# zillow/salve

Hardware: AMD Instinct MI355X
Metric: alignment hypotheses/sec (render+verify) (higher is better)
Workload: dtype fp16

## Files before the change

### salve_amd/csrc/bev_render.hip

```cpp
#include <hip/hip_runtime.h>
#include <stdlib.h>
#include <stdint.h>
#include <stdio.h>
#include <string.h>

#include "../../include/salve_hip.h"
#if defined(SALVE_PROFILE_WALK)
enum { SDC_apex = 0, SDC_apex_slow, SDC_apex_far, SDC_rows, SDC_bits, SDC_exact, SDC_apex_table, SDC_apex_cached, SDC_N };
__shared__ int sd_counters[SDC_N];
#if defined(SALVE_PROFILE_NO_COUNT)
#define SD_COUNT(c)
#else
#define SD_COUNT(c) atomicAdd(&sd_counters[SDC_##c], 1)
#endif
enum { SDP_table = 0, SDP_window, SDP_share, SDP_slow, SDP_far, SDP_e2_total, SDP_e1_total, SDP_nearest, SDP_N };
__shared__ int sd_timers[SDP_N];
__shared__ int sd_phase[8];
#define SD_HARD_REASON(slot) atomicAdd(&sd_phase[slot], 1)
#define SD_PHASE(slot, t) { const long long now_ = clock64(); if ((threadIdx.x & 63) == 0) atomicAdd(&sd_phase[slot], (int)((now_ - (t)) >> 4)); (t) = now_; }
#define SD_NOW() clock64()
#define SD_LAP(slot, t) { const long long now_ = clock64(); if ((threadIdx.x & 63) == 0) atomicAdd(&sd_timers[SDP_##slot], (int)((now_ - (t)) >> 4)); (t) = now_; }
#endif
#include "star_delaunay.h"
#include "star_local.h"
#include "star_table.h"
#include <mutex>
#include "salve_common.h"

namespace {

constexpr int DENSIFY_THREADS = 512;
constexpr int MASK_ROWS_PER_TASK = 16;
constexpr int MASK_MAX_HALF = 8;
constexpr int N_SCAL = 24;
#ifndef SALVE_E2_GROUP
#define SALVE_E2_GROUP 64
#endif
#ifndef SALVE_HARD_RUN
#define SALVE_HARD_RUN 8
#endif
constexpr int E2_GROUP = SALVE_E2_GROUP;
constexpr int HARD_RUN = SALVE_HARD_RUN;
constexpr int KEY_SLICE_SHIFT = 21;
constexpr uint32_t KEY_INDEX_MASK = (1u << KEY_SLICE_SHIFT) - 1u;

struct DevCfg {
    int pano_h, pano_w, crop_rows, rows, npts;
    int H, W, wpr, mask_half;
    float depth_scale;
    double xmin, xmax, ymin, ymax, tx, ty, scale;
    double rp00, rp01, rp10, rp11;
    double zlo[2], zhi[2], zmin;
    int nslices;
    int out_flags;
    int dbg_flags;
};

struct DensifyCfg {
    int H, W, wpr, mask_half, out_flags, dbg_flags;
};

#include "bev_splat.h"

__global__ __launch_bounds__(256) void bev_scatter_points_kernel(DevCfg c, const double* __restrict__ xyz, int npts,
                                                                 uint32_t* __restrict__ kimg, int* __restrict__ n_in_window) {
    const int i = blockIdx.x * 256 + threadIdx.x;
    if (i >= npts) return;
    const double x1 = xyz[3 * (size_t)i], y1 = xyz[3 * (size_t)i + 1], z = xyz[3 * (size_t)i + 2];
    if (!(c.xmin <= x1 && x1 <= c.xmax && c.ymin <= y1 && y1 <= c.ymax)) return;
    atomicAdd(n_in_window, 1);
    const int ix = (int)rint((x1 + c.tx) * c.scale);
    const int iy = (int)rint((y1 + c.ty) * c.scale);
    const double zs = floor(z) - c.zmin;
    if (!(zs >= 0.0 && zs < (double)c.nslices) || ix < 0 || ix >= c.W || iy < 0 || iy >= c.H) return;
    atomicMax(kimg + (size_t)iy * c.W + ix, ((uint32_t)((int)zs + 1) << KEY_SLICE_SHIFT) | (uint32_t)i);
}

struct RasterEmit {
    int H, W, wpr;
    const uint32_t* occ;
    const uint32_t* msk;
    uint32_t* bev;
    int flip;
    int lane, nlanes;
    bool skip;
    int32_t* status;
    __device__ __forceinline__ uint32_t pix(int x, int y) const { return (uint32_t)(((flip >= 0 ? flip - y : y) * W) + x); }

    static __device__ __forceinline__ int floor_div(int n, int d, float inv_d) {
        int q = (int)floorf((float)n * inv_d);
        const int r = n - q * d;
        q += (r >= d) ? 1 : 0;
        q -= (r < 0) ? 1 : 0;
        return q;
    }

    static __device__ __forceinline__ uint32_t blend(int32_t wa, int32_t wb, int32_t wc, int32_t area, float inv_area, uint32_t ca,
                                                     uint32_t cb, uint32_t cc) {
        uint32_t out = 0;
#pragma unroll
        for (int ch = 0; ch < 3; ch++) {
            const uint32_t num = __umul24((uint32_t)wa, (ca >> (8 * ch)) & 255u) + __umul24((uint32_t)wb, (cb >> (8 * ch)) & 255u) +
                                 __umul24((uint32_t)wc, (cc >> (8 * ch)) & 255u);
            uint32_t q = (uint32_t)((float)num * inv_area);
            const int32_t r = (int32_t)(num - __umul24(q, (uint32_t)area));
            q += (r >= area) ? 1u : 0u;
            q -= (r < 0) ? 1u : 0u;
            out |= q << (8 * ch);
        }
        return out;
    }

    __device__ __forceinline__ void operator()(int ax, int ay, int bx, int by, int cx, int cy) const {
        const int32_t area = sd_orient(ax, ay, bx, by, cx, cy);
        if (area <= 1 || skip) return;
        int x0 = min(ax, min(bx, cx)), x1 = max(ax, max(bx, cx));
        const int y0 = min(ay, min(by, cy)), y1 = max(ay, max(by, cy));
        if ((x0 | y0) < 0 || x1 >= W || y1 >= H) {
            if (status && lane == 0) atomicOr(status, SALVE_STATUS_WALK_FAILED);
            return;
        }
        uint32_t ca = 0, cb = 0, cc = 0;
        bool have = false;
        const bool wide = (x1 - x0) > 40;
        const float inv_area = 1.0f / (float)area;
        const int ex[3][4] = {{bx, by, cx, cy}, {cx, cy, ax, ay}, {ax, ay, bx, by}};
        int eA[3], eB[3], eC[3];
        float einv[3];
#pragma unroll
        for (int e = 0; e < 3; e++) {
            const int px = ex[e][0], py = ex[e][1], qx = ex[e][2], qy = ex[e][3];
            eA[e] = -(qy - py);
            eB[e] = qx - px;
            eC[e] = (qy - py) * px - (qx - px) * py;
            einv[e] = eA[e] != 0 ? 1.0f / (float)(eA[e] < 0 ? -eA[e] : eA[e]) : 0.f;
        }
        for (int y = y0 + lane; y <= y1; y += nlanes) {
            int xa = x0, xb = x1;
            if (wide) {
                bool empty = false;
#pragma unroll
                for (int e = 0; e < 3; e++) {
                    const int32_t A = eA[e];
                    const int32_t D = eB[e] * y + eC[e];
                    if (A > 0) {
                        xa = max(xa, floor_div(-D + A - 1, A, einv[e]));
                    } else if (A < 0) {
                        xb = min(xb, floor_div(D, -A, einv[e]));
                    } else if (D < 0) {
                        empty = true;
                    }
                }
                if (empty || xa > xb) continue;
            }
            for (int w = xa >> 5; w <= (xb >> 5); w++) {
                uint32_t bits = msk[(y * wpr) + w] & ~occ[(y * wpr) + w];
                const int lo = xa - (w << 5), hi = xb - (w << 5);
                if (lo > 0) bits &= 0xFFFFFFFFu << lo;
                if (hi < 31) bits &= 0xFFFFFFFFu >> (31 - hi);
                while (bits) {
                    const int x = (w << 5) + (__ffs((int)bits) - 1);
                    bits &= bits - 1;
                    const int32_t wa = sd_orient(bx, by, cx, cy, x, y);
                    const int32_t wb = sd_orient(cx, cy, ax, ay, x, y);
                    const int32_t wc = area - wa - wb;
                    if ((wa | wb | wc) < 0) continue;
                    if (!have) {
                        ca = __hip_atomic_load(bev + pix(ax, ay), __ATOMIC_RELAXED, __HIP_MEMORY_SCOPE_AGENT);
                        cb = __hip_atomic_load(bev + pix(bx, by), __ATOMIC_RELAXED, __HIP_MEMORY_SCOPE_AGENT);
                        cc = __hip_atomic_load(bev + pix(cx, cy), __ATOMIC_RELAXED, __HIP_MEMORY_SCOPE_AGENT);
                        have = true;
                    }
                    bev[pix(x, y)] = blend(wa, wb, wc, area, inv_area, ca, cb, cc);
                }
            }
        }
    }
};

template <class T>
__device__ __forceinline__ void store_wb(T* p, T v) { *p = v; }

constexpr uint32_t HARD_FRESH = 1u << 22;
constexpr uint32_t HARD_SECOND = 1u << 23;
__device__ __forceinline__ void push_hard(uint32_t* list, int* counter, int cap, uint32_t site, uint32_t state, int32_t* status) {
    const int k = atomicAdd(counter, 1);
    if (k < cap) {
        *reinterpret_cast<uint2*>(list + 2 * k) = make_uint2(site, state);
    } else if (status) {
        atomicOr(status, SALVE_STATUS_WALK_FAILED);
    }
}

struct QueueEmit {
    unsigned long long* queue;
    int* counter;
    int capacity;
    bool drop;
    int32_t* status;
    __device__ __forceinline__ void operator()(int ax, int ay, int bx, int by, int cx, int cy) const {
        if (drop) return;
        const int32_t area = sd_orient(ax, ay, bx, by, cx, cy);
        if (area <= 1) return;
        const int slot = atomicAdd(counter, 1);
        if (slot < capacity) {
            const uint32_t rel = (uint32_t)((bx - ax) & 0xFF) | ((uint32_t)((by - ay) & 0xFF) << 8) |
                                 ((uint32_t)((cx - ax) & 0xFF) << 16) | ((uint32_t)((cy - ay) & 0xFF) << 24);
            store_wb(queue + slot, ((unsigned long long)rel << 32) | ((uint32_t)ay << 16) | (uint32_t)ax);
        } else if (status) {
            atomicOr(status, SALVE_STATUS_WALK_FAILED);
        }
    }
};

__device__ __forceinline__ void wg_barrier_after_global_stores() {
    asm volatile("s_waitcnt vmcnt(0)" ::: "memory");
    __syncthreads();
}

__device__ __forceinline__ uint16_t f32_to_f16(float f) { return __builtin_bit_cast(uint16_t, (_Float16)f); }
__device__ __forceinline__ void tile_pixel(const uint32_t* __restrict__ img, int W, const int4 cy, const int4 cx, const float* __restrict__ lut, float v[3]) {
    const uint32_t p00 = img[(size_t)cy.x * W + cx.x], p01 = img[(size_t)cy.x * W + cx.y];
    const uint32_t p10 = img[(size_t)cy.y * W + cx.x], p11 = img[(size_t)cy.y * W + cx.y];
#pragma unroll
    for (int ch = 0; ch < 3; ch++) {
        const int a = (p00 >> (8 * ch)) & 255, b = (p01 >> (8 * ch)) & 255;
        const int cc = (p10 >> (8 * ch)) & 255, d = (p11 >> (8 * ch)) & 255;
        const int S0 = a * cx.z + b * cx.w;
        const int S1 = cc * cx.z + d * cx.w;
        int r = (((cy.z * (S0 >> 4)) >> 16) + ((cy.w * (S1 >> 4)) >> 16) + 2) >> 2;
        r = min(max(r, 0), 255);
        v[ch] = lut[ch * 256 + r];
    }
}


struct TileFuse {
    const salve_tile_job_t* jobs_a;
    const salve_tile_job_t* jobs_b;
    const uint32_t* tiles_b;
    const int32_t* coef_y;
    const int32_t* coef_x;
    const float* lut;
    uint16_t* out;
    int32_t resize, crop, out_c, reserved;
};
__global__ void bev_tile_fuse_kernel(TileFuse t, TileFuse* dst) { *dst = t; }

__device__ SdTable d_star_table;

static int ensure_star_table() {
    static std::mutex mu;
    static unsigned long long uploaded = 0;
    static SdTable host_table;
    static int built = 0;
    std::lock_guard<std::mutex> lock(mu);
    int dev = 0;
    SALVE_HIP_CHECK(hipGetDevice(&dev));
    if (dev >= 0 && dev < 64 && ((uploaded >> dev) & 1ull)) return SALVE_OK;
    if (built == 0) built = sdt_build(&host_table) ? 1 : -1;
    if (built < 0) { salve_fail("star table construction could not be certified"); return SALVE_ERR_UNSUPPORTED; }
    SALVE_HIP_CHECK(hipMemcpyToSymbol(HIP_SYMBOL(d_star_table), &host_table, sizeof(SdTable)));
    if (dev >= 0 && dev < 64) uploaded |= 1ull << dev;
    return SALVE_OK;
}

__host__ __device__ inline size_t bitmap_words_hw(int H, int W) {
    return (size_t)2 * ((W + TILE_W - 1) / TILE_W) * ((H + TILE_H - 1) / TILE_H) * TILE_H * TILE_WORDS;
}
constexpr int DENSIFY_ORDERED = 256;
constexpr int DENSIFY_TILES = 512;
__host__ __device__ inline size_t tile_fuse_word(size_t n) { return (2 * n + 3) & ~(size_t)3; }
constexpr int ORDER_BINS = 1024;
constexpr int ORDER_MIN_RENDERS = 1025;

__global__ __launch_bounds__(1024) void bev_order_kernel(const int32_t* __restrict__ cost, int n, int32_t* __restrict__ order) {
// ... 131 lines not shown
#pragma unroll
        for (int off = 1; off < 64; off <<= 1) {
            const int v = __shfl_up(incl, off);
            if (lane >= off) incl += v;
        }
        if (lane == 63) list_wave_total[wave] = incl;
        __syncthreads();
        int base = incl - cnt;
        for (int w = 0; w < wave; w++) base += list_wave_total[w];
        if (tid == DENSIFY_THREADS - 1) scal[14] = base + cnt;
        for (int i = w_begin; i < w_end; i++) {
            uint32_t bits = sdl_walk_word(occ, H, wpr, i);
            const int y = i / wpr, xb = (i - y * wpr) << 5;
            while (bits) {
                const int x = xb + __ffs((int)bits) - 1;
                bits &= bits - 1u;
                store_wb(sitelist + base++, ((uint32_t)y << 16) | (uint32_t)x);
            }
        }
    }

    {
        const int ntask_rows = (H + MASK_ROWS_PER_TASK - 1) / MASK_ROWS_PER_TASK;
        const int ntasks = ntask_rows * wpr;
        uint32_t rows[MASK_ROWS_PER_TASK + 2 * MASK_MAX_HALF];
        const bool active = tid < ntasks;
        const int w = tid % wpr, yb = (tid / wpr) * MASK_ROWS_PER_TASK;
#pragma unroll
        for (int i = 0; i < MASK_ROWS_PER_TASK + 2 * MASK_MAX_HALF; i++) {
            const int y = yb - MASK_MAX_HALF + i;
            rows[i] = (active && y >= 0 && y < H && i >= MASK_MAX_HALF - p && i < MASK_ROWS_PER_TASK + MASK_MAX_HALF + p)
                          ? msk[y * wpr + w]
                          : 0u;
        }
        __syncthreads();
#pragma unroll
        for (int i = 0; i < MASK_ROWS_PER_TASK; i++) {
            const int y = yb + i;
            uint32_t v = 0;
#pragma unroll
            for (int d = -MASK_MAX_HALF; d <= MASK_MAX_HALF; d++)
                if (d >= -p && d <= p) v |= rows[i + MASK_MAX_HALF + d];
            if (active && y < H) msk[y * wpr + w] = v;
        }
    }
    __syncthreads();

    if (c.out_flags & 2) {
        for (int i = tid; i < H * wpr; i += DENSIFY_THREADS) msk[i] = 0xFFFFFFFFu;
        __syncthreads();
    }
    const int nsites = scal[14];
    const bool degenerate = scal[0] < 4 || scal[1] == scal[2] || scal[3] <= 1;

    wg_barrier_after_global_stores();
    __builtin_amdgcn_fence(__ATOMIC_ACQUIRE, "agent");

#if defined(SALVE_PROFILE_WALK)
    SD_PHASE(0, t_phase);
#endif
    if (!degenerate && !(dbg_flags & 1)) {
        SdGrid g = {H, W, wpr, occ, rmin, rmax, 0, 1, (dbg_flags & 32) ? nullptr : &d_star_table.off[0][0][0], scal[1], scal[2], scal[12], scal[13], (H <= 1024 && W <= 1024 && !(dbg_flags & 256)) ? tri_cache : nullptr};
        RasterEmit raster = {H, W, wpr, occ, msk, bev, flip, 0, 1, (dbg_flags & 2) != 0, status};
        QueueEmit qemit = {triq, &scal[8], H * W, (dbg_flags & 1024) != 0, status};
        const int hard_cap = (H * W) >> 1;
        SdLean st;
        bool active = false, exhausted = false;
        int iters = 0;
        for (;;) {
            const unsigned long long idle = __ballot(!active && !exhausted);
            const unsigned long long busy = __ballot(active);
            if (idle != 0ull && (__popcll(idle) >= 16 || busy == 0ull)) {
                if (!active && !exhausted) {
                    const int i = atomicAdd(&scal[6], 1);
                    if (i >= nsites) {
                        exhausted = true;
                    } else {
                        const uint32_t s = __hip_atomic_load(sitelist + i, __ATOMIC_RELAXED, __HIP_MEMORY_SCOPE_AGENT);
                        if (dbg_stats) { atomicAdd(&scal[9], 1); atomicAdd(&scal[10], (int)(s & 0xFFFFu) + (int)(s >> 16)); }
                        if (sdl_lean_begin(st, g, (int)(s & 0xFFFFu), (int)(s >> 16)) == SDL_LEAN_CONTINUE) active = true;
                        else push_hard(hardlist, &scal[7], hard_cap, s, HARD_FRESH, status);
                    }
                }
            } else if (busy == 0ull) {
                break;
            }
            if (active) {
                const int r = sdl_lean_step(st, g, qemit);
                iters++;
                if (r != SDL_LEAN_CONTINUE) {
                    active = false;
                    if (dbg_mask && (dbg_flags & 16))
                    {
                        dbg_mask[((size_t)rid * H + st.sy) * W + st.sx] = (uint8_t)((r == SDL_LEAN_HARD ? 200 : 100) + min(st.deg, 50));
                    }
                    if (r == SDL_LEAN_HARD)
                        push_hard(hardlist, &scal[7], hard_cap, ((uint32_t)st.sy << 16) | (uint32_t)st.sx,
                                  (uint32_t)((st.ax + 128) & 0xFF) | ((uint32_t)((st.ay + 128) & 0xFF) << 8) | ((uint32_t)(st.n0x + 1) << 16) |
                                      ((uint32_t)(st.n0y + 1) << 18) | (st.dir > 0 ? 1u << 20 : 0u) | (st.half ? 1u << 21 : 0u) | (st.dir & 1 ? 0u : HARD_SECOND), status);
                }
            }
        }
        if (dbg_stats) atomicAdd(&scal[4], iters);
#if defined(SALVE_PROFILE_WALK)
        SD_PHASE(5, t_phase);
#endif
        wg_barrier_after_global_stores();
#if defined(SALVE_PROFILE_WALK)
        SD_PHASE(1, t_phase);
#endif
        const int nhard = min(scal[7], hard_cap);
        const int nq = min(scal[8], H * W);
        int err = 0;
#if defined(SALVE_PROFILE_WALK)
        long long t_e2 = SD_NOW();
#endif
        {
            SdGrid gw = g;
            gw.lane = lane & (E2_GROUP - 1);
            gw.nlanes = E2_GROUP;
            gw.gbase = lane & ~(E2_GROUP - 1);
            RasterEmit rw = raster;
            rw.lane = gw.lane;
            rw.nlanes = E2_GROUP;
            const int nh = (dbg_flags & 4) ? 0 : nhard;
            for (;;) {
                int i0 = 0;
                if (gw.lane == 0) i0 = atomicAdd(&scal[11], HARD_RUN);
                i0 = __shfl(i0, gw.gbase);
                if (i0 >= nh) break;
                static_assert(2 * HARD_RUN <= E2_GROUP, "a run's entries are fetched by one load of the group");
                uint32_t run_words = 0;
                if (gw.lane < 2 * HARD_RUN && 2 * i0 + gw.lane < 2 * nh)
                    run_words = __hip_atomic_load(hardlist + 2 * i0 + gw.lane, __ATOMIC_RELAXED, __HIP_MEMORY_SCOPE_AGENT);
                for (int i = i0; i < min(i0 + HARD_RUN, nh); i++) {
                    const uint32_t s = (uint32_t)__shfl((int)run_words, gw.gbase + 2 * (i - i0));
                    const uint32_t w = (uint32_t)__shfl((int)run_words, gw.gbase + 2 * (i - i0) + 1);
                    const int hx = (int)(s & 0xFFFFu), hy = (int)(s >> 16);
                    const int r = sd_walk(gw, hx, hy, (w & HARD_FRESH) != 0, (int)(w & 0xFF) - 128, (int)((w >> 8) & 0xFF) - 128, ((w >> 20) & 1u ? 1 : -1) * ((w & HARD_SECOND) ? 2 : 1),
                                          ((w >> 21) & 1u) != 0, (int)((w >> 16) & 3u) - 1, (int)((w >> 18) & 3u) - 1, rw);
                    if (r < 0) err = 1;
                }
            }
        }
#if defined(SALVE_PROFILE_WALK)
        SD_LAP(e2_total, t_e2);
        SD_PHASE(2, t_phase);
#endif
        if (err) {
            atomicOr(&scal[5], 1);
            if (status && (lane & (E2_GROUP - 1)) == 0) atomicOr(status, SALVE_STATUS_WALK_FAILED);
        }
        uint32_t* genlist = sitelist;
        for (int i = tid; i < ((dbg_flags & 8) ? 0 : nq); i += DENSIFY_THREADS) {
            const unsigned long long e = __hip_atomic_load(triq + i, __ATOMIC_RELAXED, __HIP_MEMORY_SCOPE_AGENT);
            const int ax = (int)(e & 0xFFFFu), ay = (int)((e >> 16) & 0xFFFFu);
            const uint32_t rel = (uint32_t)(e >> 32);
            const int bx = ax + (int8_t)(rel & 0xFF), by = ay + (int8_t)((rel >> 8) & 0xFF), cx = ax + (int8_t)((rel >> 16) & 0xFF), cy = ay + (int8_t)(rel >> 24);
            const int32_t area = sd_orient(ax, ay, bx, by, cx, cy);
            const bool centroid = area == 3 && (ax + bx + cx) % 3 == 0 && (ay + by + cy) % 3 == 0;
            if (area != 2 && !centroid) {
                store_wb(genlist + atomicAdd(&scal[15], 1), (uint32_t)i);
                continue;
            }
            if (dbg_flags & 2) continue;
            if (area == 2) {
                int px = cx, py = cy, qx = ax, qy = ay;
                if ((((bx - ax) | (by - ay)) & 1) == 0) { px = ax; py = ay; qx = bx; qy = by; }
                else if ((((cx - bx) | (cy - by)) & 1) == 0) { px = bx; py = by; qx = cx; qy = cy; }
                const int mx = (px + qx) >> 1, my = (py + qy) >> 1;
                if (!(((msk[(my * wpr) + (mx >> 5)] & ~occ[(my * wpr) + (mx >> 5)]) >> (mx & 31)) & 1u)) continue;
                const uint32_t cp = __hip_atomic_load(bev + pixi(px, py), __ATOMIC_RELAXED, __HIP_MEMORY_SCOPE_AGENT);
                const uint32_t cq = __hip_atomic_load(bev + pixi(qx, qy), __ATOMIC_RELAXED, __HIP_MEMORY_SCOPE_AGENT);
                bev[pixi(mx, my)] = (((cp & 0xFEFEFEu) >> 1) + ((cq & 0xFEFEFEu) >> 1) + (cp & cq & 0x010101u));
            } else {
                const int mx = (ax + bx + cx) / 3, my = (ay + by + cy) / 3;
                if (!(((msk[(my * wpr) + (mx >> 5)] & ~occ[(my * wpr) + (mx >> 5)]) >> (mx & 31)) & 1u)) continue;
                const uint32_t ca = __hip_atomic_load(bev + pixi(ax, ay), __ATOMIC_RELAXED, __HIP_MEMORY_SCOPE_AGENT);
                const uint32_t cb = __hip_atomic_load(bev + pixi(bx, by), __ATOMIC_RELAXED, __HIP_MEMORY_SCOPE_AGENT);
                const uint32_t cc = __hip_atomic_load(bev + pixi(cx, cy), __ATOMIC_RELAXED, __HIP_MEMORY_SCOPE_AGENT);
                uint32_t out = 0;
#pragma unroll
                for (int ch = 0; ch < 3; ch++) {
                    const uint32_t sum = ((ca >> (8 * ch)) & 255u) + ((cb >> (8 * ch)) & 255u) + ((cc >> (8 * ch)) & 255u);
                    out |= ((sum * 0xAAABu) >> 17) << (8 * ch);
                }
                bev[pixi(mx, my)] = out;
            }
        }
        wg_barrier_after_global_stores();
        const int ngen = min(scal[15], H * W);
        for (int i = tid; i < ngen; i += DENSIFY_THREADS) {
            const uint32_t qi = __hip_atomic_load(genlist + i, __ATOMIC_RELAXED, __HIP_MEMORY_SCOPE_AGENT);
            const unsigned long long e = __hip_atomic_load(triq + qi, __ATOMIC_RELAXED, __HIP_MEMORY_SCOPE_AGENT);
            const int ax = (int)(e & 0xFFFFu), ay = (int)((e >> 16) & 0xFFFFu);
            const uint32_t rel = (uint32_t)(e >> 32);
            raster(ax, ay, ax + (int8_t)(rel & 0xFF), ay + (int8_t)((rel >> 8) & 0xFF), ax + (int8_t)((rel >> 16) & 0xFF),
                   ay + (int8_t)(rel >> 24));
        }
    }
    wg_barrier_after_global_stores();
#if defined(SALVE_PROFILE_WALK)
    SD_PHASE(3, t_phase);
#endif
    for (int i = tid; i < H * wpr; i += DENSIFY_THREADS) {
        uint32_t bits = occ[i] & (degenerate ? 0xFFFFFFFFu : ~msk[i]);
        const int y = i / wpr, xb = (i % wpr) << 5;
        while (bits) {
            const int x = xb + __ffs((int)bits) - 1;
            bits &= bits - 1u;
            bev[pixi(x, y)] = 0u;
        }
    }
    if (c.out_flags & DENSIFY_TILES) {
        wg_barrier_after_global_stores();
        asm volatile("buffer_inv sc1" ::: "memory");
        const TileFuse* tfp = reinterpret_cast<const TileFuse*>(reinterpret_cast<const int32_t*>(bitmaps_all + (size_t)gridDim.x * bitmap_words_hw(H, W)) + tile_fuse_word(gridDim.x));
        const TileFuse tf = *tfp;
        const salve_tile_job_t ja = tf.jobs_a[rid], jb = tf.jobs_b[rid];
        if (ja.slot >= 0) {
            int4* cy_l = reinterpret_cast<int4*>(smem);
            int4* cx_l = cy_l + tf.resize;
            float* lut_l = reinterpret_cast<float*>(cx_l + tf.resize);
            for (int i = tid; i < tf.resize; i += DENSIFY_THREADS) {
                cy_l[i] = reinterpret_cast<const int4*>(tf.coef_y)[i];
                cx_l[i] = reinterpret_cast<const int4*>(tf.coef_x)[i];
            }
            for (int i = tid; i < 3 * 256; i += DENSIFY_THREADS) lut_l[i] = tf.lut[i];
            __syncthreads();
            const int crop = tf.crop, off = (tf.resize - crop) / 2, out_c = tf.out_c;
            const bool a_first = ja.chan < jb.chan;
            const int c0 = a_first ? ja.chan : jb.chan;
            const uint32_t* tb = tf.tiles_b + jb.bev_offset;
            uint16_t* osample = tf.out + (size_t)ja.slot * crop * crop * out_c;
            constexpr int COLS = 256, RGROUPS = DENSIFY_THREADS / COLS;
            for (int j0 = 0; j0 < crop; j0 += COLS) {
                const int j = j0 + (tid & (COLS - 1));
                if (j >= crop) continue;
                const int4 cx = cx_l[j + off];
#ifndef SALVE_TILE_ROWS_IN_FLIGHT
#define SALVE_TILE_ROWS_IN_FLIGHT 8
#endif
                constexpr int U = SALVE_TILE_ROWS_IN_FLIGHT;
                for (int i0 = tid / COLS; i0 < crop; i0 += RGROUPS * U) {
                    int4 cy[U];
                    uint32_t p00[U], p01[U], p10[U], p11[U], q[U];
#pragma unroll
                    for (int u = 0; u < U; u++) {
                        const int i = min(i0 + u * RGROUPS, crop - 1);
                        cy[u] = cy_l[i + off];
                        const uint32_t* r0 = bev + __umul24(cy[u].x, W);
                        const uint32_t* r1 = bev + __umul24(cy[u].y, W);
                        p00[u] = r0[cx.x]; p01[u] = r0[cx.y]; p10[u] = r1[cx.x]; p11[u] = r1[cx.y];
                        q[u] = tb[i * crop + j];
                    }
#pragma unroll
                    for (int u = 0; u < U; u++) {
                        const int i = i0 + u * RGROUPS;
                        if (i >= crop) break;
                        const int idx = i * crop + j;
                        float va[3], vb[3];
#pragma unroll
                        for (int ch = 0; ch < 3; ch++) {
                            const uint32_t a = (p00[u] >> (8 * ch)) & 255u, b = (p01[u] >> (8 * ch)) & 255u;
                            const uint32_t cc = (p10[u] >> (8 * ch)) & 255u, d = (p11[u] >> (8 * ch)) & 255u;
                            const int S0 = (int)(__umul24(a, cx.z) + __umul24(b, cx.w));
                            const int S1 = (int)(__umul24(cc, cx.z) + __umul24(d, cx.w));
                            int r = (int)(((__umul24(cy[u].z, S0 >> 4) >> 16) + (__umul24(cy[u].w, S1 >> 4) >> 16) + 2u) >> 2);
                            r = min(max(r, 0), 255);
                            va[ch] = lut_l[ch * 256 + r];
                            vb[ch] = lut_l[ch * 256 + ((q[u] >> (8 * ch)) & 255u)];
                        }
                        const float* lo = a_first ? va : vb;
                        const float* hi = a_first ? vb : va;
                        typedef float f2 __attribute__((ext_vector_type(2)));
                        typedef _Float16 h2 __attribute__((ext_vector_type(2)));
                        const uint32_t w0 = __builtin_bit_cast(uint32_t, __builtin_convertvector((f2){lo[0], lo[1]}, h2));
                        const uint32_t w1 = __builtin_bit_cast(uint32_t, __builtin_convertvector((f2){lo[2], hi[0]}, h2));
                        const uint32_t w2 = __builtin_bit_cast(uint32_t, __builtin_convertvector((f2){hi[1], hi[2]}, h2));
                        uint16_t* px = osample + (size_t)idx * out_c;
                        if (out_c == 8) {
                            *reinterpret_cast<uint4*>(px) = make_uint4(w0, w1, w2, 0u);
                        } else {
                            uint32_t* o = reinterpret_cast<uint32_t*>(px + c0);
                            o[0] = w0; o[1] = w1; o[2] = w2;
                            if (c0 + 12 > out_c)
                                for (int k = c0 + 6; k < out_c; k += 2) *reinterpret_cast<uint32_t*>(px + k) = 0u;
                        }
                    }
                }
            }
        }
    }
    if (dbg_mask) {
        for (int i = tid; i < H * W; i += DENSIFY_THREADS) {
            const int y = i / W, x = i % W;
            dbg_mask[(size_t)rid * H * W + i] = (uint8_t)((msk[y * wpr + (x >> 5)] >> (x & 31)) & 1u);
        }
    }
    if (dbg_stats) {
        __syncthreads();
#if defined(SALVE_PROFILE_WALK)
        SD_PHASE(4, t_phase);
        __syncthreads();
        if (tid < 8) dbg_stats[rid * 8 + tid] = (dbg_flags & 128) ? sd_phase[tid] : (dbg_flags & 64) ? sd_timers[tid] : sd_counters[tid];
#else
        if (tid < 8) dbg_stats[rid * 8 + tid] = tid == 1 ? scal[9] : (tid == 2 ? scal[10] : (tid < 6 ? scal[tid] : scal[tid + 1]));
#endif
    }
}


__global__ __launch_bounds__(256) void bev_tile_kernel(const uint32_t* __restrict__ bev, int W,
                                                       const salve_tile_job_t* __restrict__ jobs,
                                                       const int32_t* __restrict__ coef_y,
                                                       const int32_t* __restrict__ coef_x, int resize, int crop,
                                                       const float* __restrict__ lut, void* __restrict__ out, int fmt,
                                                       int out_c) {
    const salve_tile_job_t job = jobs[blockIdx.y];
    const int idx = blockIdx.x * 256 + threadIdx.x;
    if (idx >= crop * crop) return;
    const int i = idx / crop, j = idx % crop;
    const int off = (resize - crop) / 2;
    const int4 cy = reinterpret_cast<const int4*>(coef_y)[i + off];
    const int4 cx = reinterpret_cast<const int4*>(coef_x)[j + off];
    const uint32_t* img = bev + job.bev_offset;
    const uint32_t p00 = img[(size_t)cy.x * W + cx.x], p01 = img[(size_t)cy.x * W + cx.y];
    const uint32_t p10 = img[(size_t)cy.y * W + cx.x], p11 = img[(size_t)cy.y * W + cx.y];
    float v[3];
    int rq[3];
#pragma unroll
    for (int ch = 0; ch < 3; ch++) {
        const int a = (p00 >> (8 * ch)) & 255, b = (p01 >> (8 * ch)) & 255;
        const int cc = (p10 >> (8 * ch)) & 255, d = (p11 >> (8 * ch)) & 255;
        const int S0 = a * cx.z + b * cx.w;
        const int S1 = cc * cx.z + d * cx.w;
        int r = (((cy.z * (S0 >> 4)) >> 16) + ((cy.w * (S1 >> 4)) >> 16) + 2) >> 2;
        r = min(max(r, 0), 255);
        rq[ch] = r;
        v[ch] = lut[ch * 256 + r];
    }
    if (fmt == SALVE_TILE_U8X4) {
        reinterpret_cast<uint32_t*>(out)[(size_t)job.slot * crop * crop + idx] = (uint32_t)rq[0] | ((uint32_t)rq[1] << 8) | ((uint32_t)rq[2] << 16);
    } else if (fmt == SALVE_TILE_F32_NCHW) {
        float* o = reinterpret_cast<float*>(out) + ((size_t)job.slot * out_c + job.chan) * crop * crop + idx;
#pragma unroll
        for (int ch = 0; ch < 3; ch++) o[(size_t)ch * crop * crop] = v[ch];
    } else {
        uint16_t* o = reinterpret_cast<uint16_t*>(out) + ((size_t)job.slot * crop * crop + idx) * out_c + job.chan;
#pragma unroll
        for (int ch = 0; ch < 3; ch++) o[ch] = f32_to_f16(v[ch]);
// ... 714 lines not shown
```

### salve_amd/csrc/star_local.h

```cpp
#pragma once
#include "star_delaunay.h"
#include "star_table.h"

#define SDL_XLO (-16)
#define SDL_NONE 0x7FFF

SD_FN uint32_t sdl_row32(const SdGrid& g, int y, int x0) {
    const bool yin = (unsigned)y < (unsigned)g.H;
    const int w0 = x0 >> 5, sh = x0 & 31;
    const bool in0 = yin & ((unsigned)w0 < (unsigned)g.wpr), in1 = yin & ((unsigned)(w0 + 1) < (unsigned)g.wpr);
    const int base = SD_MUL(yin ? y : 0, g.wpr);
    uint32_t lo = g.occ[base + (in0 ? w0 : 0)], hi = g.occ[base + (in1 ? w0 + 1 : 0)];
    lo = in0 ? lo : 0u;
    hi = in1 ? hi : 0u;
#if defined(__HIP_DEVICE_COMPILE__)
    return __builtin_amdgcn_alignbit(hi, lo, (uint32_t)sh);
#else
    return sh ? ((lo >> sh) | (hi << (32 - sh))) : lo;
#endif
}

SD_FN bool sdl_bit(const SdGrid& g, int x, int y) {
    const bool in = (unsigned)x < (unsigned)g.W && (unsigned)y < (unsigned)g.H;
    const int xi = in ? x : 0, yi = in ? y : 0;
    return in & (bool)((g.occ[SD_MUL(yi, g.wpr) + (xi >> 5)] >> (xi & 31)) & 1u);
}

SD_FN uint32_t sdl_surrounded_word(uint32_t c, uint32_t l, uint32_t r, uint32_t uc) {
    const uint32_t right = (c >> 1) | (r << 31), left = (c << 1) | (l >> 31);
    return c & right & left & uc;
}
SD_FN uint32_t sdl_walk_word(const uint32_t* occ, int H, int wpr, int i) {
    const int y = i / wpr, w = i - y * wpr;
    const uint32_t c = occ[i];
    if (c == 0u || y + 1 >= H) return c;
    const uint32_t l = w > 0 ? occ[i - 1] : 0u, r = w + 1 < wpr ? occ[i + 1] : 0u;
    return c & ~sdl_surrounded_word(c, l, r, occ[i + wpr]);
}

enum { SDL_LEAN_CONTINUE = 0, SDL_LEAN_DONE = 1, SDL_LEAN_HARD = 2 };
#ifndef SD_HARD_REASON
#define SD_HARD_REASON(slot)
#endif

struct SdLean {
    int sx, sy;
    int n0x, n0y, ax, ay;
    int dir, deg;
    int round;
    bool half;
    bool aup;
};

SD_FN int sdl_lean_begin(SdLean& s, const SdGrid& g, int sx, int sy) {
    s.sx = sx;
    s.sy = sy;
    s.deg = 0;
    s.dir = 1;
    s.round = 0;
    s.half = false;
    s.aup = false;
    s.n0x = s.n0y = s.ax = s.ay = 0;
    if (g.tab == nullptr) return SDL_LEAN_HARD;
    const uint32_t c = sdl_row32(g, sy, sx + SDL_XLO), u = sdl_row32(g, sy + 1, sx + SDL_XLO), d = sdl_row32(g, sy - 1, sx + SDL_XLO);
    const int o = 0 - SDL_XLO;
    int nx = SDL_NONE, ny = 0;
    if ((d >> (o + 1)) & 1u) { nx = 1; ny = -1; }
    if ((d >> (o - 1)) & 1u) { nx = -1; ny = -1; }
    if ((u >> (o - 1)) & 1u) { nx = -1; ny = 1; }
    if ((u >> (o + 1)) & 1u) { nx = 1; ny = 1; }
    if ((d >> o) & 1u) { nx = 0; ny = -1; }
    if ((u >> o) & 1u) { nx = 0; ny = 1; }
    if ((c >> (o - 1)) & 1u) { nx = -1; ny = 0; }
    if ((c >> (o + 1)) & 1u) { nx = 1; ny = 0; }
    s.half = ((c >> (o + 1)) & 1u) != 0;
    s.n0x = s.ax = nx;
    s.n0y = s.ay = ny;
    const bool n0up = ny > 0 || s.half;
    s.aup = n0up;
    s.dir = s.half ? 2 : ((!n0up && nx < 0) ? -1 : 1);
    return nx == SDL_NONE ? SDL_LEAN_HARD : SDL_LEAN_CONTINUE;
}

template <class Emit>
SD_FN int sdl_lean_step(SdLean& s, const SdGrid& g, Emit& emit) {
    const int ox = s.dir > 0 ? 0 : s.ax, oy = s.dir > 0 ? 0 : s.ay;
    const int vx = s.dir > 0 ? s.ax : -s.ax, vy = s.dir > 0 ? s.ay : -s.ay;
    int px = SDL_NONE, py = 0;
    if (vx >= -SDT_AMAX && vx <= SDT_AMAX && vy >= -SDT_AMAX && vy <= SDT_AMAX) {
        const uint32_t* row = (const uint32_t*)(g.tab + sdt_index(vx, vy) * (SDT_LEN * 2));
        const int bx = s.sx + ox, by = s.sy + oy;
        const int k = s.round;
        const uint32_t e0 = row[2 * k], e1 = row[2 * k + 1];
        const int x0 = (int8_t)(e0 & 0xFF), y0 = (int8_t)((e0 >> 8) & 0xFF), x1 = (int8_t)((e0 >> 16) & 0xFF), y1 = (int8_t)(e0 >> 24);
        const int x2 = (int8_t)(e1 & 0xFF), y2 = (int8_t)((e1 >> 8) & 0xFF), x3 = (int8_t)((e1 >> 16) & 0xFF), y3 = (int8_t)(e1 >> 24);
        const bool b0 = sdl_bit(g, bx + x0, by + y0), b1 = sdl_bit(g, bx + x1, by + y1);
        const bool b2 = sdl_bit(g, bx + x2, by + y2), b3 = sdl_bit(g, bx + x3, by + y3);
        if (b0 | b1 | b2 | b3) {
            px = ox + (b0 ? x0 : b1 ? x1 : b2 ? x2 : x3);
            py = oy + (b0 ? y0 : b1 ? y1 : b2 ? y2 : y3);
        } else if (k + 1 < SDT_LEAN_LEN / 4) {
            s.round = k + 1;
            return SDL_LEAN_CONTINUE;
        }
    }
    s.round = 0;
    const bool second = (s.dir & 1) == 0, aup = s.aup;
    const bool n0up = s.n0y > 0;
    const bool fin = second | (aup & !n0up);
    bool sw;
    bool up = aup;
    if (px == SDL_NONE) {
        if (!sd_side_is_empty(g, s.sx, s.sy, s.sx + s.ax, s.sy + s.ay, s.dir)) {
            SD_HARD_REASON((vx >= -SDT_AMAX && vx <= SDT_AMAX && vy >= -SDT_AMAX && vy <= SDT_AMAX) ? 7 : 6);
            return SDL_LEAN_HARD;
        }
        if (fin) return SDL_LEAN_DONE;
        sw = true;
    } else {
        const bool pup = sd_before(0, 0, px, py);
        if (aup & pup) {
            if (s.dir > 0) emit(s.sx, s.sy, s.sx + s.ax, s.sy + s.ay, s.sx + px, s.sy + py);
            else emit(s.sx, s.sy, s.sx + px, s.sy + py, s.sx + s.ax, s.sy + s.ay);
        }
        sw = aup & !pup;
        if (sw ? fin : (!second && px == s.n0x && py == s.n0y)) return SDL_LEAN_DONE;
        up = pup;
    }
    if (sw) {
        s.dir = s.dir > 0 ? -2 : 2;
        px = s.n0x;
        py = s.n0y;
        up = n0up;
    }
    s.aup = up;
    s.ax = px;
    s.ay = py;
    if (++s.deg > 64) return SDL_LEAN_HARD;
    return SDL_LEAN_CONTINUE;
}
```

Baseline: 60370.

## Batch densify and raster triangle loads to keep several in flight

Restructures the densify loop and the general-triangle raster loop so each thread handles several triangles per iteration. It issues all queue and pixel-color loads up front before doing any compute or stores, which hides global memory latency. The raster functor gains a templated path that accepts prefetched vertex colors. Separately, the lean star-walk step is rewritten with early returns to simplify control flow. The cost is higher register pressure and extra clamped or dummy loads at the loop tails.

```diff
diff --git a/salve_amd/csrc/bev_render.hip b/salve_amd/csrc/bev_render.hip
--- a/salve_amd/csrc/bev_render.hip
+++ b/salve_amd/csrc/bev_render.hip
@@ -41,6 +41,10 @@
 #endif
 constexpr int E2_GROUP = SALVE_E2_GROUP;
 constexpr int HARD_RUN = SALVE_HARD_RUN;
+#ifndef SALVE_RASTER_TRIS_IN_FLIGHT
+#define SALVE_RASTER_TRIS_IN_FLIGHT 4
+#endif
+constexpr int RASTER_TRIS = SALVE_RASTER_TRIS_IN_FLIGHT;
 constexpr int KEY_SLICE_SHIFT = 21;
 constexpr uint32_t KEY_INDEX_MASK = (1u << KEY_SLICE_SHIFT) - 1u;
 
@@ -111,7 +115,14 @@
         return out;
     }
 
-    __device__ __forceinline__ void operator()(int ax, int ay, int bx, int by, int cx, int cy) const {
+    __device__ __forceinline__ void operator()(int ax, int ay, int bx, int by, int cx, int cy) const { run<false>(ax, ay, bx, by, cx, cy, 0u, 0u, 0u); }
+
+    __device__ __forceinline__ bool inside(int ax, int ay, int bx, int by, int cx, int cy) const {
+        return (min(ax, min(bx, cx)) | min(ay, min(by, cy))) >= 0 && max(ax, max(bx, cx)) < W && max(ay, max(by, cy)) < H;
+    }
+
+    template <bool FETCHED>
+    __device__ __forceinline__ void run(int ax, int ay, int bx, int by, int cx, int cy, uint32_t ca, uint32_t cb, uint32_t cc) const {
         const int32_t area = sd_orient(ax, ay, bx, by, cx, cy);
         if (area <= 1 || skip) return;
         int x0 = min(ax, min(bx, cx)), x1 = max(ax, max(bx, cx));
@@ -120,8 +131,7 @@
             if (status && lane == 0) atomicOr(status, SALVE_STATUS_WALK_FAILED);
             return;
         }
-        uint32_t ca = 0, cb = 0, cc = 0;
-        bool have = false;
+        bool have = FETCHED;
         const bool wide = (x1 - x0) > 40;
         const float inv_area = 1.0f / (float)area;
         const int ex[3][4] = {{bx, by, cx, cy}, {cx, cy, ax, ay}, {ax, ay, bx, by}};
@@ -559,51 +569,113 @@
             if (status && (lane & (E2_GROUP - 1)) == 0) atomicOr(status, SALVE_STATUS_WALK_FAILED);
         }
         uint32_t* genlist = sitelist;
-        for (int i = tid; i < ((dbg_flags & 8) ? 0 : nq); i += DENSIFY_THREADS) {
-            const unsigned long long e = __hip_atomic_load(triq + i, __ATOMIC_RELAXED, __HIP_MEMORY_SCOPE_AGENT);
-            const int ax = (int)(e & 0xFFFFu), ay = (int)((e >> 16) & 0xFFFFu);
-            const uint32_t rel = (uint32_t)(e >> 32);
-            const int bx = ax + (int8_t)(rel & 0xFF), by = ay + (int8_t)((rel >> 8) & 0xFF), cx = ax + (int8_t)((rel >> 16) & 0xFF), cy = ay + (int8_t)(rel >> 24);
-            const int32_t area = sd_orient(ax, ay, bx, by, cx, cy);
-            const bool centroid = area == 3 && (ax + bx + cx) % 3 == 0 && (ay + by + cy) % 3 == 0;
-            if (area != 2 && !centroid) {
-                store_wb(genlist + atomicAdd(&scal[15], 1), (uint32_t)i);
-                continue;
-            }
-            if (dbg_flags & 2) continue;
-            if (area == 2) {
-                int px = cx, py = cy, qx = ax, qy = ay;
-                if ((((bx - ax) | (by - ay)) & 1) == 0) { px = ax; py = ay; qx = bx; qy = by; }
-                else if ((((cx - bx) | (cy - by)) & 1) == 0) { px = bx; py = by; qx = cx; qy = cy; }
-                const int mx = (px + qx) >> 1, my = (py + qy) >> 1;
+        constexpr int U = RASTER_TRIS;
+        enum { TRI_NONE = 0, TRI_MIDPOINT = 1, TRI_CENTROID = 2, TRI_GENERAL = 3 };
+        const int nqf = (dbg_flags & 8) ? 0 : nq;
+        for (int i0 = tid; i0 < nqf; i0 += U * DENSIFY_THREADS) {
+            unsigned long long e[U];
+#pragma unroll
+            for (int u = 0; u < U; u++) {
+                const int i = i0 + u * DENSIFY_THREADS;
+                e[u] = __hip_atomic_load(triq + min(i, nqf - 1), __ATOMIC_RELAXED, __HIP_MEMORY_SCOPE_AGENT);
+            }
+            int kind[U];
+            uint32_t ca[U], cb[U], cc[U], dst[U];
+#pragma unroll
+            for (int u = 0; u < U; u++) {
+                const int ax = (int)(e[u] & 0xFFFFu), ay = (int)((e[u] >> 16) & 0xFFFFu);
+                const uint32_t rel = (uint32_t)(e[u] >> 32);
+                const int bx = ax + (int8_t)(rel & 0xFF), by = ay + (int8_t)((rel >> 8) & 0xFF), cx = ax + (int8_t)((rel >> 16) & 0xFF), cy = ay + (int8_t)(rel >> 24);
+                const int32_t area = sd_orient(ax, ay, bx, by, cx, cy);
+                const bool centroid = area == 3 && (ax + bx + cx) % 3 == 0 && (ay + by + cy) % 3 == 0;
+                kind[u] = TRI_NONE;
+                ca[u] = cb[u] = cc[u] = dst[u] = 0u;
+                if (i0 + u * DENSIFY_THREADS >= nqf) continue;
+                if (area != 2 && !centroid) {
+                    kind[u] = TRI_GENERAL;
+                    continue;
+                }
+                if (dbg_flags & 2) continue;
+                int mx, my;
+                if (area == 2) {
+                    int px = cx, py = cy, qx = ax, qy = ay;
+                    if ((((bx - ax) | (by - ay)) & 1) == 0) { px = ax; py = ay; qx = bx; qy = by; }
+                    else if ((((cx - bx) | (cy - by)) & 1) == 0) { px = bx; py = by; qx = cx; qy = cy; }
+                    mx = (px + qx) >> 1; my = (py + qy) >> 1;
+                    ca[u] = pixi(px, py); cb[u] = pixi(qx, qy);
+                } else {
+                    mx = (ax + bx + cx) / 3; my = (ay + by + cy) / 3;
+                    ca[u] = pixi(ax, ay); cb[u] = pixi(bx, by); cc[u] = pixi(cx, cy);
+                }
                 if (!(((msk[(my * wpr) + (mx >> 5)] & ~occ[(my * wpr) + (mx >> 5)]) >> (mx & 31)) & 1u)) continue;
-                const uint32_t cp = __hip_atomic_load(bev + pixi(px, py), __ATOMIC_RELAXED, __HIP_MEMORY_SCOPE_AGENT);
-                const uint32_t cq = __hip_atomic_load(bev + pixi(qx, qy), __ATOMIC_RELAXED, __HIP_MEMORY_SCOPE_AGENT);
-                bev[pixi(mx, my)] = (((cp & 0xFEFEFEu) >> 1) + ((cq & 0xFEFEFEu) >> 1) + (cp & cq & 0x010101u));
-            } else {
-                const int mx = (ax + bx + cx) / 3, my = (ay + by + cy) / 3;
-                if (!(((msk[(my * wpr) + (mx >> 5)] & ~occ[(my * wpr) + (mx >> 5)]) >> (mx & 31)) & 1u)) continue;
-                const uint32_t ca = __hip_atomic_load(bev + pixi(ax, ay), __ATOMIC_RELAXED, __HIP_MEMORY_SCOPE_AGENT);
-                const uint32_t cb = __hip_atomic_load(bev + pixi(bx, by), __ATOMIC_RELAXED, __HIP_MEMORY_SCOPE_AGENT);
-                const uint32_t cc = __hip_atomic_load(bev + pixi(cx, cy), __ATOMIC_RELAXED, __HIP_MEMORY_SCOPE_AGENT);
-                uint32_t out = 0;
+                kind[u] = area == 2 ? TRI_MIDPOINT : TRI_CENTROID;
+                dst[u] = pixi(mx, my);
+            }
+#pragma unroll
+            for (int u = 0; u < U; u++) {
+                if (kind[u] == TRI_MIDPOINT || kind[u] == TRI_CENTROID) {
+                    ca[u] = __hip_atomic_load(bev + ca[u], __ATOMIC_RELAXED, __HIP_MEMORY_SCOPE_AGENT);
+                    cb[u] = __hip_atomic_load(bev + cb[u], __ATOMIC_RELAXED, __HIP_MEMORY_SCOPE_AGENT);
+                }
+                if (kind[u] == TRI_CENTROID) cc[u] = __hip_atomic_load(bev + cc[u], __ATOMIC_RELAXED, __HIP_MEMORY_SCOPE_AGENT);
+            }
+            uint32_t out[U];
+#pragma unroll
+            for (int u = 0; u < U; u++) {
+                const uint32_t mid = (((ca[u] & 0xFEFEFEu) >> 1) + ((cb[u] & 0xFEFEFEu) >> 1) + (ca[u] & cb[u] & 0x010101u));
+                uint32_t third = 0;
 #pragma unroll
                 for (int ch = 0; ch < 3; ch++) {
-                    const uint32_t sum = ((ca >> (8 * ch)) & 255u) + ((cb >> (8 * ch)) & 255u) + ((cc >> (8 * ch)) & 255u);
-                    out |= ((sum * 0xAAABu) >> 17) << (8 * ch);
+                    const uint32_t sum = ((ca[u] >> (8 * ch)) & 255u) + ((cb[u] >> (8 * ch)) & 255u) + ((cc[u] >> (8 * ch)) & 255u);
+                    third |= ((sum * 0xAAABu) >> 17) << (8 * ch);
                 }
-                bev[pixi(mx, my)] = out;
+                out[u] = kind[u] == TRI_CENTROID ? third : mid;
+                asm volatile("" : "+v"(out[u]));
+            }
+#pragma unroll
+            for (int u = 0; u < U; u++) {
+                if (kind[u] == TRI_GENERAL) store_wb(genlist + atomicAdd(&scal[15], 1), (uint32_t)(i0 + u * DENSIFY_THREADS));
+                else if (kind[u] != TRI_NONE) bev[dst[u]] = out[u];
             }
         }
         wg_barrier_after_global_stores();
         const int ngen = min(scal[15], H * W);
-        for (int i = tid; i < ngen; i += DENSIFY_THREADS) {
-            const uint32_t qi = __hip_atomic_load(genlist + i, __ATOMIC_RELAXED, __HIP_MEMORY_SCOPE_AGENT);
-            const unsigned long long e = __hip_atomic_load(triq + qi, __ATOMIC_RELAXED, __HIP_MEMORY_SCOPE_AGENT);
-            const int ax = (int)(e & 0xFFFFu), ay = (int)((e >> 16) & 0xFFFFu);
-            const uint32_t rel = (uint32_t)(e >> 32);
-            raster(ax, ay, ax + (int8_t)(rel & 0xFF), ay + (int8_t)((rel >> 8) & 0xFF), ax + (int8_t)((rel >> 16) & 0xFF),
-                   ay + (int8_t)(rel >> 24));
+        for (int i0 = tid; i0 < ngen; i0 += U * DENSIFY_THREADS) {
+            uint32_t qi[U];
+            unsigned long long e[U];
+            uint32_t ca[U], cb[U], cc[U];
+#pragma unroll
+            for (int u = 0; u < U; u++)
+                qi[u] = __hip_atomic_load(genlist + min(i0 + u * DENSIFY_THREADS, ngen - 1), __ATOMIC_RELAXED, __HIP_MEMORY_SCOPE_AGENT);
+#pragma unroll
+            for (int u = 0; u < U; u++) e[u] = __hip_atomic_load(triq + qi[u], __ATOMIC_RELAXED, __HIP_MEMORY_SCOPE_AGENT);
+#pragma unroll
+            for (int u = 0; u < U; u++)
+                if (i0 + u * DENSIFY_THREADS >= ngen) e[u] = 0ull;
+#pragma unroll
+            for (int u = 0; u < U; u++) {
+                const int ax = (int)(e[u] & 0xFFFFu), ay = (int)((e[u] >> 16) & 0xFFFFu);
+                const uint32_t rel = (uint32_t)(e[u] >> 32);
+                const int bx = ax + (int8_t)(rel & 0xFF), by = ay + (int8_t)((rel >> 8) & 0xFF), cx = ax + (int8_t)((rel >> 16) & 0xFF), cy = ay + (int8_t)(rel >> 24);
+                ca[u] = cb[u] = cc[u] = 0u;
+                if (i0 + u * DENSIFY_THREADS < ngen && raster.inside(ax, ay, bx, by, cx, cy)) {
+                    ca[u] = __hip_atomic_load(bev + raster.pix(ax, ay), __ATOMIC_RELAXED, __HIP_MEMORY_SCOPE_AGENT);
+                    cb[u] = __hip_atomic_load(bev + raster.pix(bx, by), __ATOMIC_RELAXED, __HIP_MEMORY_SCOPE_AGENT);
+                    cc[u] = __hip_atomic_load(bev + raster.pix(cx, cy), __ATOMIC_RELAXED, __HIP_MEMORY_SCOPE_AGENT);
+                }
+            }
+#pragma unroll 1
+            for (int u = 0; u < U; u++) {
+                unsigned long long eu = e[0];
+                uint32_t cau = ca[0], cbu = cb[0], ccu = cc[0];
+#pragma unroll
+                for (int k = 1; k < U; k++)
+                    if (u == k) { eu = e[k]; cau = ca[k]; cbu = cb[k]; ccu = cc[k]; }
+                const int ax = (int)(eu & 0xFFFFu), ay = (int)((eu >> 16) & 0xFFFFu);
+                const uint32_t rel = (uint32_t)(eu >> 32);
+                raster.run<true>(ax, ay, ax + (int8_t)(rel & 0xFF), ay + (int8_t)((rel >> 8) & 0xFF), ax + (int8_t)((rel >> 16) & 0xFF),
+                                 ay + (int8_t)(rel >> 24), cau, cbu, ccu);
+            }
         }
     }
     wg_barrier_after_global_stores();
diff --git a/salve_amd/csrc/star_local.h b/salve_amd/csrc/star_local.h
--- a/salve_amd/csrc/star_local.h
+++ b/salve_amd/csrc/star_local.h
@@ -4,6 +4,9 @@
 
 #define SDL_XLO (-16)
 #define SDL_NONE 0x7FFF
+#ifndef SALVE_LEAN_EARLY_RETURN
+#define SALVE_LEAN_EARLY_RETURN 1
+#endif
 
 SD_FN uint32_t sdl_row32(const SdGrid& g, int y, int x0) {
     const bool yin = (unsigned)y < (unsigned)g.H;
@@ -108,6 +111,36 @@
     const bool second = (s.dir & 1) == 0, aup = s.aup;
     const bool n0up = s.n0y > 0;
     const bool fin = second | (aup & !n0up);
+#if SALVE_LEAN_EARLY_RETURN
+    if (px == SDL_NONE) {
+        if (!sd_side_is_empty(g, s.sx, s.sy, s.sx + s.ax, s.sy + s.ay, s.dir)) {
+            SD_HARD_REASON((vx >= -SDT_AMAX && vx <= SDT_AMAX && vy >= -SDT_AMAX && vy <= SDT_AMAX) ? 7 : 6);
+            return SDL_LEAN_HARD;
+        }
+        if (fin) return SDL_LEAN_DONE;
+    } else {
+        const bool pup = sd_before(0, 0, px, py);
+        if (aup & pup) {
+            if (s.dir > 0) emit(s.sx, s.sy, s.sx + s.ax, s.sy + s.ay, s.sx + px, s.sy + py);
+            else emit(s.sx, s.sy, s.sx + px, s.sy + py, s.sx + s.ax, s.sy + s.ay);
+        }
+        if (!(aup & !pup)) {
+            if (!second && px == s.n0x && py == s.n0y) return SDL_LEAN_DONE;
+            s.aup = pup;
+            s.ax = px;
+            s.ay = py;
+            if (++s.deg > 64) return SDL_LEAN_HARD;
+            return SDL_LEAN_CONTINUE;
+        }
+        if (fin) return SDL_LEAN_DONE;
+    }
+    s.dir = s.dir > 0 ? -2 : 2;
+    s.aup = n0up;
+    s.ax = s.n0x;
+    s.ay = s.n0y;
+    if (++s.deg > 64) return SDL_LEAN_HARD;
+    return SDL_LEAN_CONTINUE;
+#else
     bool sw;
     bool up = aup;
     if (px == SDL_NONE) {
@@ -138,4 +171,5 @@
     s.ay = py;
     if (++s.deg > 64) return SDL_LEAN_HARD;
     return SDL_LEAN_CONTINUE;
+#endif
 }
```

Measured after the change: 60860 (median of 6 runs). Within noise of the previous version (+0.8%).
